# lambdaclass/mina_bridge

Measured on AMD Instinct MI355X. Metric: Mina state proofs verified/sec (batch), higher is better.
Workload: dtype u32x8-montgomery (255-bit prime fields, integer)

## Files before the change

### bindings/go/minaverify.go

```go
package minaverify

import "C"

import (
	"errors"
	"unsafe"
)

type Ctx struct{ p *C.mina_ctx }

func lastError() error { return errors.New(C.GoString(C.mina_last_error())) }

func New(device int) (*Ctx, error) {
	var p *C.mina_ctx
	if rc := C.mina_ctx_create(C.int(device), &p); rc != 0 {
		return nil, lastError()
	}
	return &Ctx{p}, nil
}

func (c *Ctx) Close() { C.mina_ctx_destroy(c.p) }

func (c *Ctx) SrsCreate(curve int, depth uint32) error {
	if rc := C.mina_srs_create(c.p, C.int(curve), C.uint32_t(depth)); rc != 0 {
// ... 18 lines not shown
	if rc := C.mina_ctx_state_dedup_stats(c.p, &a, &b, &d); rc != 0 {
		return 0, 0, 0, lastError()
	}
	return uint64(a), uint64(b), uint64(d), nil
}

func ConfigureDedupStates(otherFlags uint32) { C.mina_verify_configure(C.uint32_t(otherFlags) | C.MINA_VERIFY_DEDUP_STATES) }

func ConfigurePackOnDevice(otherFlags uint32) { C.mina_verify_configure(C.uint32_t(otherFlags) | C.MINA_VERIFY_PACK_ON_DEVICE) }

func ConfigureAccountOnDevice(otherFlags uint32) { C.mina_verify_configure(C.uint32_t(otherFlags) | C.MINA_VERIFY_ACCOUNT_ON_DEVICE) }

func ConfigureGroupedSearch(otherFlags uint32) { C.mina_verify_configure(C.uint32_t(otherFlags) | C.MINA_VERIFY_GROUPED_SEARCH) }

func (c *Ctx) SetSearchGroups(groups uint32) error {
	if rc := C.mina_ctx_set_search_groups(c.p, C.uint32_t(groups)); rc != 0 {
		return lastError()
	}
	return nil
}

func (c *Ctx) SetStreamBudget(n int) error {
	if rc := C.mina_ctx_set_stream_budget(c.p, C.int(n)); rc != 0 {
		return lastError()
	}
	return nil
}

func (c *Ctx) SearchStats() (searches, rounds, parts uint64, err error) {
	var a, b, d C.uint64_t
	if rc := C.mina_ctx_search_stats(c.p, &a, &b, &d); rc != 0 {
		return 0, 0, 0, lastError()
	}
	return uint64(a), uint64(b), uint64(d), nil
}

func (c *Ctx) StateJobEachDev(jobs *C.mina_state_jobs, dVerdicts, dFlags unsafe.Pointer) error {
	if rc := C.mina_state_job_each_dev(c.p, jobs, dVerdicts, dFlags); rc != 0 {
		return lastError()
	}
	return nil
}

func (c *Ctx) MsmSegmentsDev(curve int, nTotal, nseg int, dBegin, dEnd, dBases, dScalars, dOut unsafe.Pointer) error {
	if rc := C.mina_msm_segments_dev(c.p, C.int(curve), C.size_t(nTotal), C.size_t(nseg), dBegin, dEnd, dBases, dScalars, dOut); rc != 0 {
		return lastError()
// ... 78 lines not shown
```

### bindings/rust/src/sys.rs

```rust
#![allow(non_camel_case_types)]
use std::os::raw::{c_char, c_int, c_void};

#[repr(C)] pub struct mina_ctx { _private: [u8; 0] }

#[repr(C)]
pub struct mina_ipa_opening {
    pub k: u32,
    pub lr: *const u8,
    pub delta: *const u8,
    pub sg: *const u8,
    pub z1: *const u8,
    pub z2: *const u8,
    pub n_evalpoints: u32,
    pub evalpoints: *const u8,
    pub n_comms: u32,
    pub comms: *const u8,
    pub combined_inner_product: *const u8,
    pub polyscale: *const u8,
    pub evalscale: *const u8,
    pub sponge_state: *const u8,
    pub sponge_mode: u32,
    pub sponge_count: u32,
}

// ... 256 lines not shown
    pub fn mina_verify_account_inclusion(ctx: *mut mina_ctx, n: usize, proofs: *const *const u8, proof_lens: *const usize, pub_inputs: *const *const u8, pub_lens: *const usize, leaf_hashes: *const u8, verdicts: *mut u8) -> c_int;
    pub fn mina_consensus_project_window(p: *const mina_consensus_params, s: *const mina_consensus_state, next_global_slot: u32, out_window: *mut u32) -> c_int;
    pub fn mina_consensus_relative_min_window_density(p: *const mina_consensus_params, a: *const mina_consensus_state, b: *const mina_consensus_state, out: *mut u32) -> c_int;
    pub fn mina_consensus_is_short_range(a: *const mina_consensus_state, b: *const mina_consensus_state) -> c_int;
    pub fn mina_consensus_select_secure_chain(p: *const mina_consensus_params, tip: *const mina_consensus_state, candidate: *const mina_consensus_state, candidate_selected: *mut c_int) -> c_int;
    pub fn mina_protocol_state_pack(bytes: *const u8, len: usize, encoding: c_int, record: *mut u8, n_body_fields: *mut u32, info: *mut mina_protocol_state_info, consumed: *mut usize) -> c_int;
    pub fn mina_protocol_state_hash_batch(ctx: *mut mina_ctx, n: usize, records: *const u8, n_body_fields: *const u32, hashes_out: *mut u8, body_hashes_out: *mut u8) -> c_int;
    pub fn mina_protocol_state_dedup_dev(ctx: *mut mina_ctx, n: usize, d_records: *const c_void, d_nfields: *const c_void, d_rep: *mut c_void, d_counts: *mut c_void, fingerprint_bits: u32) -> c_int;
    pub fn mina_protocol_state_hash_batch_dedup(ctx: *mut mina_ctx, n: usize, records: *const u8, n_body_fields: *const u32, hashes_out: *mut u8, body_hashes_out: *mut u8, n_distinct: *mut usize) -> c_int;
    pub fn mina_ctx_set_state_dedup(ctx: *mut mina_ctx, on: c_int) -> c_int;
    pub fn mina_ctx_state_dedup_stats(ctx: *mut mina_ctx, states: *mut u64, distinct: *mut u64, collisions: *mut u64) -> c_int;
    pub fn mina_protocol_state_pack_dev(ctx: *mut mina_ctx, n: usize, d_blob: *const c_void, blob_len: usize, d_off: *const c_void, d_len: *const c_void, d_records: *mut c_void, d_nfields: *mut c_void, d_info: *mut c_void, d_status: *mut c_void) -> c_int;
    pub fn mina_state_frontend_dev(ctx: *mut mina_ctx, batch: usize, d_blob: *const c_void, blob_len: usize, d_begin: *const c_void, d_end: *const c_void, d_expected_hashes: *const c_void, d_ledger_hashes: *const c_void, d_and: *const c_void, d_records: *mut c_void, d_nfields: *mut c_void, d_precheck: *mut c_void, d_masks: *mut c_void) -> c_int;
    pub fn mina_protocol_state_hash_bytes(ctx: *mut mina_ctx, encoding: c_int, n: usize, states: *const *const u8, lens: *const usize, hashes_out: *mut u8) -> c_int;
    pub fn mina_state_jobs_prepare(ctx: *mut mina_ctx, log2_domain: u32, npub: u32) -> c_int;
    pub fn mina_state_job_batch_dev(ctx: *mut mina_ctx, jobs: *const mina_state_jobs, d_verdicts: *mut c_void, d_flags: *mut c_void) -> c_int;
    pub fn mina_state_job_fold_dev(ctx: *mut mina_ctx, jobs: *const mina_state_jobs, d_verdicts: *mut c_void, d_flags: *mut c_void, d_ipa_scalars: *mut c_void, d_ipa_point: *mut c_void, d_acc_scalars: *mut c_void, d_acc_point: *mut c_void) -> c_int;
    pub fn mina_state_job_batch(ctx: *mut mina_ctx, jobs: *const mina_state_jobs, verdicts: *mut u8) -> c_int;
    pub fn mina_state_job_each_dev(ctx: *mut mina_ctx, jobs: *const mina_state_jobs, d_verdicts: *mut c_void, d_flags: *mut c_void) -> c_int;
    pub fn mina_ctx_set_search_groups(ctx: *mut mina_ctx, groups: u32) -> c_int;
    pub fn mina_ctx_search_stats(ctx: *mut mina_ctx, searches: *mut u64, rounds: *mut u64, parts: *mut u64) -> c_int;
    pub fn mina_ctx_lane_streams(ctx: *mut mina_ctx, live: *mut u32, made_by_searches: *mut u64) -> c_int;
    pub fn mina_ctx_set_stream_budget(ctx: *mut mina_ctx, n: c_int) -> c_int;
    pub fn mina_challenge_to_field_dev(ctx: *mut mina_ctx, field: c_int, n: usize, d_chal128: *const c_void, d_out: *mut c_void) -> c_int;
    pub fn mina_field_sum_rows_dev(ctx: *mut mina_ctx, field: c_int, rows: usize, m: usize, d_in: *const c_void, d_out: *mut c_void) -> c_int;
    pub fn mina_msm_srs_range_dev(ctx: *mut mina_ctx, curve: c_int, first: u32, n: usize, d_scalars: *const c_void, d_out: *mut c_void) -> c_int;
    pub fn mina_msm_dev(ctx: *mut mina_ctx, curve: c_int, n: usize, d_bases: *const c_void, d_scalars: *const c_void, d_out: *mut c_void) -> c_int;
    pub fn mina_points_sum_dev(ctx: *mut mina_ctx, curve: c_int, n: usize, d_records: *const c_void, d_out: *mut c_void) -> c_int;
    pub fn mina_point_records_equal_dev(ctx: *mut mina_ctx, d_a: *const c_void, d_b: *const c_void, d_verdict: *mut c_void) -> c_int;
    pub fn mina_msm_segments_dev(ctx: *mut mina_ctx, curve: c_int, n_total: usize, nseg: usize, d_seg_begin: *const c_void, d_seg_end: *const c_void, d_bases: *const c_void, d_scalars: *const c_void, d_out: *mut c_void) -> c_int;
    pub fn mina_b_poly_fold_segments_dev(ctx: *mut mina_ctx, field: c_int, k: u32, batch: usize, nseg: usize, d_seg_begin: *const c_void, d_seg_end: *const c_void, d_chals: *const c_void, d_weights: *const c_void, d_out: *mut c_void) -> c_int;
    pub fn mina_verifier_index_install(ctx: *mut mina_ctx, index: *const mina_verifier_index) -> c_int;
    pub fn mina_verifier_index_digest(ctx: *mut mina_ctx, out32: *mut u8) -> c_int;
    pub fn mina_polish_tokens_from_json(field: c_int, json: *const c_char, len: usize, enabled_features: u32, optional_present: u32, out: *mut u8, cap: usize, out_len: *mut usize) -> c_int;
    pub fn mina_verifier_index_load_json(ctx: *mut mina_ctx, index_json: *const c_char, index_len: usize, constant_term_json: *const c_char, ct_len: usize, perm_alpha_offset: u32) -> c_int;
    pub fn mina_kimchi_to_batch(ctx: *mut mina_ctx, proofs: *const mina_kimchi_proofs, out: *mut mina_kimchi_batch_out) -> c_int;
    pub fn mina_step_index_install(ctx: *mut mina_ctx, index: *const mina_step_index) -> c_int;
    pub fn mina_step_index_load_json(ctx: *mut mina_ctx, n_indexes: usize, index_jsons: *const *const c_char, index_lens: *const usize, constant_term_json: *const c_char, ct_len: usize, enabled_features: u32, optional_present: u32) -> c_int;
    pub fn mina_pickles_public_inputs_batch(ctx: *mut mina_ctx, st: *const mina_pickles_statements, batch: usize, public_inputs_out: *mut u8, ok: *mut u8) -> c_int;
    pub fn mina_pickles_public_input(ctx: *mut mina_ctx, wrap_proof: *const u8, len: usize, encoding: c_int, app_state: *const u8, public_input_out: *mut u8, derived_out: *mut u8) -> c_int;
    pub fn mina_wrap_proof_flatten(bytes: *const u8, len: usize, encoding: c_int, out: *mut u8, cap: usize, out_len: *mut usize, consumed: *mut usize) -> c_int;
    pub fn mina_state_proof_split(bytes: *const u8, len: usize, proof_len: *mut usize, state_offsets: *mut usize, state_lens: *mut usize) -> c_int;
    pub fn mina_verify_state(proof: *const u8, proof_len: usize, pub_input: *const u8, pub_len: usize) -> bool;
    pub fn mina_verify_state_batch(n: usize, proofs: *const *const u8, proof_lens: *const usize, pub_inputs: *const *const u8, pub_lens: *const usize, verdicts_out: *mut u8) -> c_int;
    pub fn mina_verify_state_checks(proof: *const u8, proof_len: usize, pub_input: *const u8, pub_len: usize, passed_mask: *mut u32, ran_mask: *mut u32) -> c_int;
    pub fn mina_verify_state_files(proof_path: *const c_char, pub_path: *const c_char) -> bool;
// ... 30 lines not shown
```

### include/mina_verify.h

```cpp
#ifndef MINA_VERIFY_H
#define MINA_VERIFY_H

#include <stddef.h>
#include <stdint.h>

#ifdef __cplusplus
extern "C" {
#endif

#define MINA_OK 0
#define MINA_ERR_ARG (-1)
#define MINA_ERR_HIP (-2)
#define MINA_ERR_STATE (-3)
#define MINA_ERR_FORMAT (-4)

#define MINA_FIELD_FP 0
#define MINA_FIELD_FQ 1
#define MINA_CURVE_PALLAS 0
#define MINA_CURVE_VESTA 1

typedef struct mina_ctx mina_ctx;

int mina_ctx_create(int device_id, mina_ctx **out);
void mina_ctx_destroy(mina_ctx *ctx);
// ... 260 lines not shown
    const void *precheck;
    uint32_t log2_domain, npub, pub_comm_slot;
    const void *public_inputs;
    int with_ipa;
    uint32_t k, n_evalpoints, n_comms;
    const void *sponge_state , *sponge_pos , *cip , *lr , *delta ,
               *sg , *z1, *z2 , *evalpoints , *evalscale, *polyscale , *comms ;
    const void *rand_base, *sg_rand_base;
    const struct mina_kimchi_proofs *kimchi;
    int with_accumulator;
    uint32_t acc_k;
    const void *acc_prechallenges , *acc_sg , *acc_rho ;
} mina_state_jobs;
int mina_state_jobs_prepare(mina_ctx *ctx, uint32_t log2_domain, uint32_t npub);
int mina_state_job_batch_dev(mina_ctx *ctx, const mina_state_jobs *jobs, void *d_verdicts, void *d_flags);
int mina_state_job_fold_dev(mina_ctx *ctx, const mina_state_jobs *jobs, void *d_verdicts, void *d_flags, void *d_ipa_scalars, void *d_ipa_point,
                            void *d_acc_scalars, void *d_acc_point);
int mina_state_job_batch(mina_ctx *ctx, const mina_state_jobs *jobs, uint8_t *verdicts );
int mina_state_job_each_dev(mina_ctx *ctx, const mina_state_jobs *jobs, void *d_verdicts , void *d_flags );
int mina_ctx_set_search_groups(mina_ctx *ctx, uint32_t groups);
int mina_ctx_search_stats(mina_ctx *ctx, uint64_t *searches, uint64_t *rounds, uint64_t *parts);
int mina_ctx_lane_streams(mina_ctx *ctx, uint32_t *live, uint64_t *made_by_searches);
int mina_ctx_set_stream_budget(mina_ctx *ctx, int n);

int mina_challenge_to_field_dev(mina_ctx *ctx, int field, size_t n, const void *d_chal128 , void *d_out );
int mina_field_sum_rows_dev(mina_ctx *ctx, int field, size_t rows, size_t m, const void *d_in , void *d_out );
int mina_msm_srs_range_dev(mina_ctx *ctx, int curve, uint32_t first, size_t n, const void *d_scalars, void *d_out );
int mina_msm_dev(mina_ctx *ctx, int curve, size_t n, const void *d_bases , const void *d_scalars , void *d_out );
int mina_points_sum_dev(mina_ctx *ctx, int curve, size_t n, const void *d_records , void *d_out );
int mina_point_records_equal_dev(mina_ctx *ctx, const void *d_a, const void *d_b, void *d_verdict );
int mina_msm_segments_dev(mina_ctx *ctx, int curve, size_t n_total, size_t nseg, const void *d_seg_begin, const void *d_seg_end ,
                          const void *d_bases , const void *d_scalars , void *d_out );
int mina_b_poly_fold_segments_dev(mina_ctx *ctx, int field, uint32_t k, size_t batch, size_t nseg, const void *d_seg_begin,
                                  const void *d_seg_end , const void *d_chals ,
                                  const void *d_weights , void *d_out );

struct mina_pickles_statements;
#define MINA_TOK_ALPHA 0
#define MINA_TOK_BETA 1
#define MINA_TOK_GAMMA 2
#define MINA_TOK_JOINT_COMBINER 3
#define MINA_TOK_ENDO_COEFFICIENT 4
#define MINA_TOK_MDS 5
#define MINA_TOK_LITERAL 6
#define MINA_TOK_CELL 7
#define MINA_TOK_DUP 8
// ... 188 lines not shown
```

### mina_bridge_amd/csrc/api_core.hip

```cpp
#include "ctx.h"
#include "sponge.cuh"
#include "msm.cuh"

#include <sys/random.h>
#include <atomic>
#include <condition_variable>
#include <deque>
#include <mutex>

template <int F> static fe_t host_modulus() { fe_t p; for (int i = 0; i < 8; ++i) p.v[i] = modulus_limb<F>(i); return p; }
static void fe_shr1(fe_t &a) { for (int i = 0; i < 7; ++i) a.v[i] = (a.v[i] >> 1) | (a.v[i + 1] << 31); a.v[7] >>= 1; }
static fe_t fe_sub_small(const fe_t &a, uint32_t k) { fe_t r = a; uint64_t br = k; for (int i = 0; i < 8 && br; ++i) { uint64_t t = (uint64_t)r.v[i] - br; r.v[i] = (uint32_t)t; br = (t >> 32) & 1u; } return r; }
static fe_t fe_div3(const fe_t &a) { fe_t r; uint64_t rem = 0; for (int i = 7; i >= 0; --i) { uint64_t cur = (rem << 32) | a.v[i]; r.v[i] = (uint32_t)(cur / 3); rem = cur % 3; } return r; }

template <int F> static FieldK make_field_consts() {
    FieldK k;
    fe_t p = host_modulus<F>();
    fe_t a = fe_zero(); a.v[0] = 1;
    for (int i = 0; i < 512; ++i) { a = fe_add<F>(a, a); if (i == 255) k.one = a; }
    k.r2 = a;
    fe_t pm1 = fe_sub_small(p, 1);
    k.pm2 = fe_sub_small(p, 2);
    k.pm1d2 = pm1; fe_shr1(k.pm1d2);
    k.half = k.pm1d2;
// ... 65 lines not shown
    if (v->step_host && v->step_host_free && v->step_host != p->step_host) v->step_host_free(v->step_host);
    v->step_host = p->step_host; v->step_host_free = nullptr;
    v->state_salts.alias(p->state_salts); v->have_state_salts = p->have_state_salts;
}

extern "C" void mina_ctx_destroy(mina_ctx *c) {
    if (!c) return;
    (void)hipSetDevice(c->device);
    for (int i = 0; i < MB_DEV_HELPER0; ++i) if (c->lanes[i].stream) (void)hipStreamSynchronize(c->lanes[i].stream);
    for (hipStream_t s : c->fork_own) if (s) (void)hipStreamSynchronize(s);
    for (hipStream_t s : c->role) if (s) (void)hipStreamSynchronize(s);
    for (int i = 0; i < 2; ++i) { c->srs[i].table.release(); c->srs[i].table29.release(); c->srs[i].table29s.release(); c->srs[i].h.release(); c->srs[i].lagrange_table.release(); c->srs[i].lagrange_digits.release(); c->srs[i].lagrange_digits29.release(); c->pparams[i].release(); c->merkle_salts[i].release(); }
    c->state_salts.release(); c->acct_defaults.release(); c->dedup_totals.release(); c->kimchi_index.release(); c->kimchi_tokens.release(); c->kimchi_literals.release();
    c->pickles_index.release(); c->pickles_tokens.release(); c->pickles_literals.release();
    if (c->step_host && c->step_host_free) c->step_host_free(c->step_host);
    c->step_host = nullptr;
    for (int i = 0; i < MB_MAX_LANES; ++i) c->lanes[i].release_all();
    for (auto &r : c->prof.recs) { (void)hipEventDestroy(r.a); (void)hipEventDestroy(r.b); }
    for (int i = 0; i < MB_MAX_LANES; ++i) {
        Lane &L = c->lanes[i];
        if (L.aux) { (void)hipStreamSynchronize(L.aux); (void)hipStreamDestroy(L.aux); (void)hipEventDestroy(L.ev_fork); (void)hipEventDestroy(L.ev_join); }
        if (L.ev_leg) (void)hipEventDestroy(L.ev_leg);
        if (L.ev_done) (void)hipEventDestroy(L.ev_done);
        if (L.stream && i < MB_DEV_HELPER0) (void)hipStreamDestroy(L.stream);
    }
    for (hipStream_t s : c->fork_own) if (s) (void)hipStreamDestroy(s);
    for (hipStream_t s : c->role) if (s) (void)hipStreamDestroy(s);
    delete c;
}

__attribute__((constructor)) static void mb_default_hw_queues() { setenv("GPU_MAX_HW_QUEUES", "16", 0); }

extern "C" int mina_ctx_synchronize(mina_ctx *c) {
    if (!c) return fail(MINA_ERR_ARG, "null ctx");
    HIPC(hipSetDevice(c->device));
    HIPC(mb_ctx_wait_all(c));
    return MINA_OK;
}
extern "C" int mina_ctx_set_stream_budget(mina_ctx *c, int n) {
    if (!c) return fail(MINA_ERR_ARG, "null ctx");
    if (n > 31) return fail(MINA_ERR_ARG, "stream budget: at most 31 (32 hardware queues less the null stream's); <= 0 = the environment's");
    HIPC(hipSetDevice(c->device));
    HIPC(mb_ctx_wait_all(c));
    c->stream_budget = n > 0 ? n : 0;
    return MINA_OK;
}
extern "C" void *mina_ctx_stream(mina_ctx *c) { return c ? (void *)c->lanes[c->pinned >= 0 ? c->pinned : 0].stream : nullptr; }
extern "C" int mina_ctx_pin_lane(mina_ctx *c, int lane) {
    if (!c) return fail(MINA_ERR_ARG, "null ctx");
    if (lane >= c->nlanes) return fail(MINA_ERR_ARG, "lane outside the pipeline (mina_ctx_set_pipeline)");
    c->pinned = lane < 0 ? -1 : lane;
    return MINA_OK;
}

extern "C" int mina_ctx_set_pipeline(mina_ctx *c, int lanes) {
    if (!c) return fail(MINA_ERR_ARG, "null ctx");
    if (lanes < 1 || lanes > MB_PIPE_LANES) return fail(MINA_ERR_ARG, "lanes must be in 1..32");
    HIPC(hipSetDevice(c->device));
    HIPC(mb_ctx_wait_all(c));
    for (int i = 0; i < lanes; ++i)
        if (!c->lanes[i].stream) HIPC(hipStreamCreateWithFlags(&c->lanes[i].stream, hipStreamNonBlocking));
    c->nlanes = lanes; c->rr = 0; c->pinned = -1; c->use_lane0();
    return MINA_OK;
}

extern "C" int mina_to_group(mina_ctx *c, int curve, size_t n, const uint8_t *t, uint8_t *out) {
    if (!c || (n && (!t || !out))) return fail(MINA_ERR_ARG, "null argument");
// ... 180 lines not shown
```

### mina_bridge_amd/csrc/api_state.hip

```cpp
#include <chrono>
#include <optional>
#include "ctx.h"
#include "msm.cuh"
#include "sponge.cuh"
#include "lagrange.cuh"
#include "wire_state.h"
#include "state_dedup.cuh"

namespace mb {

template <int F> __device__ __forceinline__ fe_t ld_fe(const uint32_t *p) { fe_t r; for (int i = 0; i < 8; ++i) r.v[i] = p[i]; return r; }

template <int F, int LANES>
__device__ __forceinline__ void pstate_sponge(const bool live, const bool writer, const uint32_t e, const uint32_t sp, const uint32_t *__restrict__ rec, const uint32_t nf,
                                              const FieldK &fk, const PoseidonParams *__restrict__ pp, const fe_t *__restrict__ salts, uint32_t *__restrict__ out_hash,
                                              uint32_t *__restrict__ out_body) {
#if defined(__HIP_DEVICE_COMPILE__)
    if constexpr (LANES == 3) {
        const TriPos tp = tri_pos();
        const PoseidonParams29 *__restrict__ q = pparams29_of(pp);
        auto field29 = [&](const uint32_t *w, bool take) {
            fe_t v = fe_zero();
            if (take) v = ld_fe<F>(w);
            return fe29_mul_sg<F>(fe29_from_words(v), q->absorb);
// ... 186 lines not shown
static int ensure_state_salts(mina_ctx *c) {
    if (c->have_state_salts) return MINA_OK;
    if (!c->have_pparams[FIELD_FP]) return fail(MINA_ERR_STATE, "Poseidon constants not installed for Fp");
    const char *names[MB_N_PREFIX_SALTS] = {"MinaProtoStateBody", "MinaProtoState", "MinaAccount", "MinaZkappAccount", "MinaZkappUri", "MinaSideLoadedVk"};
    uint8_t pre[MB_N_PREFIX_SALTS * 32];
    for (int i = 0; i < MB_N_PREFIX_SALTS; ++i) { const mw::B32 f = mw::prefix_field(names[i]); memcpy(pre + 32 * i, f.b, 32); }
    int rc;
    if ((rc = c->state_salts.ensure(MB_N_PREFIX_SALTS * 3 * sizeof(fe_t)))) return rc;
    DevBuf tmp;
    if ((rc = tmp.ensure(sizeof pre))) return rc;
    HIPC(hipMemcpyAsync(tmp.p, pre, sizeof pre, hipMemcpyHostToDevice, c->L->stream));
    mb::prefix_salt_kernel<FIELD_FP><<<1, 64, 0, c->L->stream>>>(MB_N_PREFIX_SALTS, c->fk[FIELD_FP], c->pparams[FIELD_FP].as<PoseidonParams>(), tmp.as<uint32_t>(), c->state_salts.as<fe_t>());
    HIPC(hipGetLastError());
    HIPC(hipStreamSynchronize(c->L->stream));
    tmp.release();
    c->have_state_salts = true;
    return MINA_OK;
}

int mb_ensure_state_salts(mina_ctx *c) { return ensure_state_salts(c); }

struct UniqList { const uint32_t *m, *uniq; };
static int pstate_hash_launch(mina_ctx *c, size_t n, size_t leg, HashLaunch hl, const uint32_t *d_records, const uint32_t *d_nfields, uint32_t *d_hashes, uint32_t *d_bodies,
                              const UniqList *u) {
    const PoseidonParams *pp = c->pparams[FIELD_FP].as<PoseidonParams>();
    const fe_t *salts = c->state_salts.as<fe_t>();
    hipStream_t stream = c->L->stream;
    return with_lanes<1, 16, 8, 3>(pstate_hash_lanes(c, n, leg), [&](auto lanes) {
        constexpr int LN = decltype(lanes)::value;
        constexpr bool wide = LN == 1 || LN == 3;
        std::optional<ProfScope> ps1_;
        if (LN == 1) ps1_.emplace(c, PS_STATE_HASH1);
        const size_t per = wide && hl.piece_waves ? hash_piece_states(c, leg, hl.piece_waves) : n;
        const uint32_t lds = wide ? hl.lds_bytes : 0;
        for (size_t lo = 0; lo < n; lo += per) {
            const size_t cnt = std::min(per, n - lo);
            const uint32_t grid = cdiv(coop_threads<LN>(cnt), 256);
            if (u) {
                if constexpr (LN == 1) mb::pstate_hash1_uniq_kernel<FIELD_FP><<<grid, 256, lds, stream>>>((uint32_t)lo, (uint32_t)cnt, u->m, u->uniq, pp, salts, d_records, d_nfields, d_hashes, d_bodies);
                else mb::pstate_hash_uniq_kernel<FIELD_FP, LN><<<grid, 256, lds, stream>>>((uint32_t)lo, (uint32_t)cnt, u->m, u->uniq, c->fk[FIELD_FP], pp, salts, d_records, d_nfields, d_hashes, d_bodies);
                continue;
            }
            const uint32_t *rec = d_records + lo * MINA_PSTATE_SLOTS * 8, *nf = d_nfields + lo;
            uint32_t *hash = d_hashes + lo * 8, *body = d_bodies ? d_bodies + lo * 8 : nullptr;
            if constexpr (LN == 1) mb::pstate_hash1_kernel<FIELD_FP><<<grid, 256, lds, stream>>>((uint32_t)cnt, pp, salts, rec, nf, hash, body);
            else mb::pstate_hash_kernel<FIELD_FP, LN><<<grid, 256, lds, stream>>>((uint32_t)cnt, c->fk[FIELD_FP], pp, salts, rec, nf, hash, body);
        }
        HIPC(hipGetLastError());
        return MINA_OK;
    });
}

static int pstate_hash_dev(mina_ctx *c, size_t n, size_t leg, HashLaunch hl, const uint32_t *d_records, const uint32_t *d_nfields, uint32_t *d_hashes, uint32_t *d_bodies) {
    ProfScope ps_(c, PS_STATE_HASH);
    return pstate_hash_launch(c, n, leg, hl, d_records, d_nfields, d_hashes, d_bodies, nullptr);
}
// ... 193 lines not shown
    if (!LS || lo + cnt > ns_total) return fail(MINA_ERR_ARG, "bad early state range");
    if (!c->have_state_salts) return fail(MINA_ERR_STATE, "call mina_state_jobs_prepare first");
    if (!LS->stream) HIPC(hipStreamCreateWithFlags(&LS->stream, hipStreamNonBlocking));
    int rc;
    if ((rc = LS->st_hashes.ensure(ns_total * 32))) return rc;
    if (after) HIPC(hipStreamWaitEvent(LS->stream, after, 0));
    Lane *const L0 = c->L;
    c->L = LS;
    rc = pstate_hash_dev(c, cnt, ns_total, hash, d_records + lo * MINA_PSTATE_SLOTS * 8, d_nfields + lo, LS->st_hashes.as<uint32_t>() + lo * 8, nullptr);
    c->L = L0;
    return rc;
}


static int state_leg(mina_ctx *c, const mina_state_jobs *j, Lane &S, const StateJobPlan &plan) {
    c->L = &S;
    const size_t B = j->batch;
    int rc;
    if (j->with_states) {
        const size_t ns = B * MINA_STATES_PER_PROOF;
        if ((rc = S.st_hashes.ensure(ns * 32))) return rc;
        const size_t early = std::min(plan.hashed_early, ns);
        const uint32_t *rec = (const uint32_t *)j->state_records, *nf = (const uint32_t *)j->state_nfields;
        if (c->state_dedup && early == 0) {
            if ((rc = pstate_hash_dedup_dev(c, ns, ns, plan.hash, rec, nf, S.st_hashes.as<uint32_t>(), nullptr, true))) return rc;
        } else if (early < ns && (rc = pstate_hash_dev(c, ns - early, ns, plan.hash, rec + early * MINA_PSTATE_SLOTS * 8, nf + early, S.st_hashes.as<uint32_t>() + early * 8, nullptr))) return rc;
        mb::pstate_chain_check_kernel<<<cdiv(B, 64), 64, 0, S.stream>>>((uint32_t)B, S.st_hashes.as<uint32_t>(), (const uint32_t *)j->expected_hashes, rec, (const uint8_t *)j->precheck, S.st_ok.as<uint32_t>());
    } else {
        if (j->precheck) return fail(MINA_ERR_ARG, "precheck needs the protocol-state section");
        mb::fill_u32_kernel<<<cdiv(B, 256), 256, 0, S.stream>>>((uint32_t)B, 1u, S.st_ok.as<uint32_t>());
    }
    HIPC(hipGetLastError());
    return MINA_OK;
}

static int accumulator_leg(mina_ctx *c, const mina_state_jobs *j, Lane &A, const FoldExport *fx, StateJobCarry &v) {
    c->L = &A;
    if (!j->with_accumulator) return MINA_OK;
    const size_t B = j->batch;
    int rc;
    if ((rc = A.st_flags.ensure(16 * 4))) return rc;
    v.acc_v = A.st_flags.as<uint32_t>() + 8;
    return mb_accumulator_check_dev(c, CURVE_VESTA, j->acc_k, B, (const uint32_t *)j->acc_prechallenges, (const uint32_t *)j->acc_sg, B > 1 ? (const uint32_t *)j->acc_rho : nullptr, v.acc_v, fx);
}

static int wrap_leg(mina_ctx *c, const mina_state_jobs *j, Lane &L, const FoldExport *fx, StateJobCarry &v, hipStream_t stage2 = nullptr) {
    c->L = &L;
    const size_t B = j->batch;
// ... 140 lines not shown
    const StreamPlan sp = stream_plan(in_flight, c->stream_budget > 0 ? c->stream_budget : c->stream_budget_env);
    const uint32_t mode = c->dev_fork_made ? c->dev_fork_made : tu.dev_fork;
    c->dev_fork_made = mode;
    int prio_lo = 0, prio_hi = 0;
    auto make = [&](hipStream_t &st, bool chain, bool masked, int prio) -> int {
        if (st) return MINA_OK;
        int ncu = 0; (void)hipDeviceGetAttribute(&ncu, hipDeviceAttributeMultiprocessorCount, c->device);
        if (masked && tu.dev_chain_cus > 0 && tu.dev_chain_cus < (uint32_t)ncu && ncu <= 256) {
            uint32_t mk[8] = {0, 0, 0, 0, 0, 0, 0, 0};
            for (uint32_t b2 = 0; b2 < (uint32_t)ncu; ++b2) if ((b2 < tu.dev_chain_cus) == chain) mk[b2 >> 5] |= 1u << (b2 & 31);
            if (hipExtStreamCreateWithCUMask(&st, 8, mk) == hipSuccess) return MINA_OK;
            (void)hipGetLastError(); st = nullptr;
        }
        if (prio_lo != prio_hi && (mode & 4u)) HIPC(hipStreamCreateWithPriority(&st, hipStreamNonBlocking, prio));
        else HIPC(hipStreamCreateWithFlags(&st, hipStreamNonBlocking));
        return MINA_OK;
    };
    int rc;
    if (sp.roles) {
        if (!c->role[sp.streams - 1]) (void)hipDeviceGetStreamPriorityRange(&prio_lo, &prio_hi);
        for (int i = 0; i < sp.streams; ++i) if ((rc = make(c->role[i], true, false, (i == 0 && sp.streams > 1) ? prio_lo : prio_hi))) return rc;
        plan.role_h = c->role[0]; plan.role_w1 = c->role[sp.w1(li)]; plan.role_w2 = c->role[sp.w2(li)];
        plan.wrap = &h[0]; plan.acc = &h[1]; plan.states = &h[2];
    } else {
        hipStream_t *own = &c->fork_own[3 * li];
        if (!own[0] || !own[1] || !own[2]) {
            (void)hipDeviceGetStreamPriorityRange(&prio_lo, &prio_hi);
            if ((rc = make(own[0], true, (mode & 2u) != 0, prio_hi)) || (rc = make(own[1], true, false, (prio_lo + prio_hi) / 2)) || (rc = make(own[2], false, (mode & 2u) != 0, prio_lo))) return rc;
        }
        for (int q = 0; q < 3; ++q) h[q].stream = own[q];
        if (L0.on_roles) {
            HIPC(hipStreamWaitEvent(L0.stream, L0.ev_done, 0));
            L0.on_roles = false;
        }
        plan.wrap = &h[0]; plan.acc = tu.dev_acc_lane ? &h[2] : &h[1]; plan.states = &h[2];
        plan.acc_first = tu.dev_acc_lane == 2;
    }
    uint32_t piece = tu.dev_piece_waves;
    if (piece == 0 && in_flight >= 2 && !sp.roles) piece = (hash_one_lane(c, leg_states) ? 12288u : 6144u) / (uint32_t)in_flight;
    if (piece == 0xffffffffu) piece = 0;
    plan.hash.piece_waves = piece;
    uint32_t lds_kb = tu.dev_hash_lds_kb;
    if (lds_kb == 0 && in_flight == 1) lds_kb = 41;
    if (lds_kb == 0xffffffffu || lds_kb > 160) lds_kb = 0;
    plan.hash.lds_bytes = lds_kb * 1024u;
    return MINA_OK;
// ... 272 lines not shown
```

### mina_bridge_amd/csrc/ctx.h

```cpp
#pragma once
#include <hip/hip_runtime.h>

#include <cstdio>
#include <cstdlib>
#include <cstring>
#include <array>
#include <functional>
#include <memory>
#include <mutex>
#include <thread>
#include <algorithm>
#include <string>
#include <type_traits>
#include <utility>
#include <vector>

#include "../../include/mina_verify.h"
#include "groupmap.cuh"

using namespace mb;

struct mina_ctx;
int mb_ctx_create_view(mina_ctx *parent, mina_ctx **out);
void mb_ctx_refresh_view(mina_ctx *view, mina_ctx *parent);
// ... 50 lines not shown
    int lagrange_table_log2 = -1;
    DevBuf lagrange_digits;
    uint32_t lagrange_digits_n = 0;
    DevBuf lagrange_digits29;
};

struct MsmWorkspace {
    DevBuf scalars, points, points29 , ekey, eval, eoff, count, start, task_start, rem_pos, rem_bucket, info, sorted, partial, heavy, order, redo, ghist, stage, buckets, red_r, red_ws, red2_r, red2_w, set_total, out_words, out_xyzz, buckets29, seg_bad;
};

enum ProfStage : int { PS_DIGITS = 0, PS_SCAN, PS_SCATTER, PS_ACCUMULATE, PS_BUCKET_SUM, PS_REDUCE_A, PS_REDUCE_BC, PS_FINISH,
                       PS_BPOLY_TABLES, PS_BPOLY_FOLD, PS_BPOLY_FINISH, PS_STATE_HASH, PS_IPA_TRANSCRIPT, PS_KIMCHI, PS_PICKLES,
                       PS_STATE_HASH1 , PS_COUNT };
struct ProfState {
    int mask = 0;
    struct Rec { hipEvent_t a, b; int stage; };
    std::vector<Rec> recs; size_t used = 0;
};

struct Lane {
    hipStream_t stream = nullptr;
    hipStream_t aux = nullptr;
    hipEvent_t ev_fork = nullptr, ev_join = nullptr, ev_leg = nullptr;
    hipEvent_t ev_done = nullptr; bool on_roles = false;
    MsmWorkspace ws;
    DevBuf tmp_a, tmp_b, tmp_c, tmp_d;
    PinnedBuf host_stage;
    DevBuf bp_ltab, bp_htab, bp_partial, bp_ldig, bp_hdig, bp_colsum;
    DevBuf ipa_chals, ipa_folded, ipa_xyzz_a, ipa_xyzz_b, ipa_points, ipa_scalars, ipa_sigma, ipa_in_a, ipa_in_b, ipa_in_c, ipa_verdict, ipa_xfer, ipa_shared, ipa_shared_off, acc_rho_scaled ;
    DevBuf st_ok, st_hashes, st_pub_xyzz, st_pubcomm, st_flags, st_in, st_verdicts;
    DevBuf dd_rep, dd_uniq, dd_table, dd_counts;
    DevBuf pk_off, pk_len, pk_status, pk_info, pk_fmt;
    DevBuf ac_ws, ac_in;
    DevBuf gs_tab, gs_folded, gs_xa, gs_xb, gs_chals, gs_points, gs_bad, gs_flags;
    DevBuf kc_state, kc_pos, kc_cip, kc_pts, kc_v, kc_u, kc_comms, kc_xfer, kc_pch, pk_xe, pk_pub, pk_ok;
    void release_all() {
        MsmWorkspace &w = ws;
        DevBuf *all[] = {&w.scalars, &w.points, &w.points29, &w.ekey, &w.eval, &w.eoff, &w.count, &w.start, &w.task_start, &w.rem_pos, &w.rem_bucket, &w.info, &w.sorted, &w.partial, &w.heavy, &w.order, &w.redo, &w.ghist, &w.stage,
                         &w.buckets, &w.buckets29, &w.seg_bad, &w.red_r, &w.red_ws, &w.red2_r, &w.red2_w, &w.set_total, &w.out_words, &w.out_xyzz, &tmp_a, &tmp_b, &tmp_c, &tmp_d,
                         &bp_ltab, &bp_htab, &bp_partial, &bp_ldig, &bp_hdig, &bp_colsum, &ipa_chals, &ipa_folded, &ipa_xyzz_a, &ipa_xyzz_b, &ipa_points, &ipa_scalars,
                         &ipa_sigma, &ipa_in_a, &ipa_in_b, &ipa_in_c, &ipa_verdict, &ipa_xfer, &ipa_shared, &ipa_shared_off, &acc_rho_scaled,
                         &st_ok, &st_hashes, &st_pub_xyzz, &st_pubcomm, &st_flags, &st_in, &st_verdicts,
                         &dd_rep, &dd_uniq, &dd_table, &dd_counts, &pk_off, &pk_len, &pk_status, &pk_info, &pk_fmt, &ac_ws, &ac_in,
                         &gs_tab, &gs_folded, &gs_xa, &gs_xb, &gs_chals, &gs_points, &gs_bad, &gs_flags,
                         &kc_state, &kc_pos, &kc_cip, &kc_pts, &kc_v, &kc_u, &kc_comms, &kc_xfer, &kc_pch, &pk_xe, &pk_pub, &pk_ok};
        for (DevBuf *b : all) b->release();
// ... 39 lines not shown
    DevBuf pparams[2]; bool have_pparams[2] = {false, false};
    DevBuf merkle_salts[2]; uint32_t merkle_depth[2] = {0, 0};
    DevBuf kimchi_index, kimchi_tokens, kimchi_literals; bool have_kimchi = false; uint32_t kimchi_log2 = 0; uint8_t kimchi_digest[32] = {0};
    uint8_t kimchi_comms_host[28 * 64] = {0};
    DevBuf pickles_index, pickles_tokens, pickles_literals; bool have_pickles_dev = false, pickles_ms_valid = false;
    void *step_host = nullptr; void (*step_host_free)(void *) = nullptr;
    bool pparams_surrogate[2] = {false, false};
    bool pparams_rows1[2] = {false, false};
    DevBuf state_salts; bool have_state_salts = false;
    bool is_view = false;
    bool state_dedup = false;
    DevBuf dedup_totals; uint64_t dedup_states = 0;
    int (*state_frontend)(mina_ctx *c, size_t batch, const void *d_blob, size_t blob_len, const void *d_begin, const void *d_end, const void *d_expected_hashes,
                          const void *d_ledger_hashes, const void *d_and, void *d_records, void *d_nfields, void *d_precheck, void *d_masks) = nullptr;
    DevBuf acct_defaults; bool have_acct_defaults = false;
    int (*account_on_device)(mina_ctx *c, size_t n, const uint8_t *const *proofs, const size_t *proof_lens, const uint8_t *const *pubs, const size_t *pub_lens,
                             uint32_t *passed, uint32_t *ran, Lane *lane, std::mutex *enq_mu) = nullptr;
    uint32_t search_groups = 0; uint64_t gs_searches = 0, gs_rounds = 0, gs_parts = 0;
    uint64_t search_streams_made = 0;
    int (*state_job_each)(mina_ctx *c, const mina_state_jobs *dev_jobs, uint8_t *verdicts) = nullptr;
    uint32_t dev_fork_made = 0;
    hipStream_t fork_own[3 * MB_DEV_FORK_MAX] = {}; hipStream_t role[MB_ROLE_STREAMS] = {};
    int stream_budget = 0, stream_budget_env = -1;
    void use_lane0() { L = &lanes[0]; }
    void next_lane() { L = pinned >= 0 ? &lanes[pinned] : &lanes[rr++ % (unsigned)nlanes]; }
};

static inline hipError_t mb_ctx_wait_all(mina_ctx *c) {
    for (int i = 0; i < c->nlanes; ++i) if (c->lanes[i].stream) { hipError_t e = hipStreamSynchronize(c->lanes[i].stream); if (e != hipSuccess) return e; }
    for (hipStream_t s : c->role) if (s) { hipError_t e = hipStreamSynchronize(s); if (e != hipSuccess) return e; }
    return hipSuccess;
}

static inline int mb_ctx_state_dedup(mina_ctx *c, bool on) {
    if (on && !c->state_dedup) {
        if (mb_ctx_wait_all(c) != hipSuccess) return MINA_ERR_HIP;
        int rc = c->dedup_totals.ensure(16);
        if (rc) return rc;
        if (hipMemsetAsync(c->dedup_totals.p, 0, 16, c->lanes[0].stream) != hipSuccess || hipStreamSynchronize(c->lanes[0].stream) != hipSuccess) return MINA_ERR_HIP;
        c->dedup_states = 0;
    }
    c->state_dedup = on;
    return MINA_OK;
}

static constexpr size_t COOP8_MAX_GROUPS = 8192;
static inline bool use_coop8(const mina_ctx *c, size_t groups) {
    const mina_verify_tuning t = mb_tune();
    return groups * (size_t)((c && !t.coop8_per_call) ? c->nlanes : 1) <= (size_t)t.coop8_max;
}

static inline bool use_coop16(const mina_ctx *c, size_t proofs) {
    return proofs * (size_t)(c ? c->nlanes : 1) <= (size_t)mb_tune().coop16_max;
}

static inline bool use_coop8_transcripts(const mina_ctx *c, size_t batch, size_t per_call_limit) {
    const size_t lim = (size_t)mb_tune().transcript_coop8_max;
    const size_t in_flight = batch * (size_t)(c ? c->nlanes : 1);
    return lim ? in_flight <= lim : ((batch <= per_call_limit && in_flight <= 2048) || in_flight <= 2560);
}

static constexpr size_t HASH1_MIN_STATES = 65536;
static inline int hash_jobs_in_flight(const mina_ctx *c) { return c->pinned >= 0 ? 1 : c->nlanes; }
static inline bool hash_one_lane(const mina_ctx *c, size_t leg_states) {
    const int jobs = hash_jobs_in_flight(c);
    return c->pparams_rows1[FIELD_FP] && jobs >= 2 && leg_states * (size_t)jobs >= HASH1_MIN_STATES;
}
static inline size_t hash_piece_states(const mina_ctx *c, size_t leg_states, uint32_t piece_waves) { return (size_t)piece_waves * (hash_one_lane(c, leg_states) ? 64u : 21u); }

static inline int hash_lanes(const mina_ctx *c, size_t proofs, size_t sponges) { return use_coop16(c, proofs) ? 16 : (use_coop8(c, sponges) ? 8 : 3); }
static inline int pstate_hash_lanes(const mina_ctx *c, size_t n, size_t leg_states) {
    return hash_one_lane(c, leg_states) ? 1 : hash_lanes(c, (n + MINA_STATES_PER_PROOF - 1) / MINA_STATES_PER_PROOF, n);
}
static inline int transcript_lanes(const mina_ctx *c, size_t batch, size_t per_call_limit) {
    return use_coop16(c, batch) ? 16 : (use_coop8_transcripts(c, batch, per_call_limit) ? 8 : 3);
}
static inline int sponge_batch_lanes(size_t n) { return n <= COOP8_MAX_GROUPS ? 8 : 3; }
static inline int merkle_lanes(const mina_ctx *c, size_t paths) { return use_coop16(c, paths) ? 16 : sponge_batch_lanes(paths); }

enum : uint32_t { MB_JOB_LEGS = 1, MB_JOB_FINISH = 2, MB_JOB_ALL = 3 };
struct StateJobCarry { uint32_t *ipa_v = nullptr, *acc_v = nullptr, *kimchi_bad = nullptr; const uint32_t *stmt_ok = nullptr; };
struct HashLaunch { uint32_t piece_waves = 0, lds_bytes = 0; };
struct FoldExport { uint32_t *ipa_scalars = nullptr, *ipa_point = nullptr, *acc_scalars = nullptr, *acc_point = nullptr; };
struct StateJobPlan {
    Lane *wrap = nullptr, *acc = nullptr, *states = nullptr;
    uint32_t phase = MB_JOB_ALL; StateJobCarry *carry = nullptr;
    uint32_t *d_stmt_out = nullptr;
    size_t hashed_early = 0;
    HashLaunch hash;
    bool acc_first = false;
    hipStream_t role_h = nullptr, role_w1 = nullptr, role_w2 = nullptr;
    const FoldExport *fold_export = nullptr;
};
int mb_state_jobs_on_lane(mina_ctx *c, const mina_state_jobs *j, uint32_t *d_verdicts, uint32_t *d_flags, const StateJobPlan &plan = {});
int mb_verify_account_on(mina_ctx *c, size_t n, const uint8_t *const *proofs, const size_t *proof_lens, const uint8_t *const *pubs, const size_t *pub_lens,
                         uint32_t *passed, uint32_t *ran, Lane *lane, std::mutex *enq_mu);
int mb_state_frontend_on_lane(mina_ctx *c, size_t batch, const void *d_blob, size_t blob_len, const void *d_begin, const void *d_end, const void *d_expected_hashes,
                              const void *d_ledger_hashes, const void *d_and, void *d_records, void *d_nfields, void *d_precheck, void *d_masks);
int mb_verify_account_dev_on(mina_ctx *c, size_t n, const uint8_t *const *proofs, const size_t *proof_lens, const uint8_t *const *pubs, const size_t *pub_lens,
                             uint32_t *passed, uint32_t *ran, Lane *lane, std::mutex *enq_mu);
int mb_state_job_each_host(mina_ctx *c, const mina_state_jobs *dev_jobs, uint8_t *verdicts);
int mb_state_hashes_early(mina_ctx *c, Lane *LS, size_t ns_total, size_t lo, size_t cnt, const uint32_t *d_records, const uint32_t *d_nfields, hipEvent_t after, HashLaunch hash);

struct MbPoolJob;
std::shared_ptr<MbPoolJob> mb_pool_submit(size_t n, std::function<void(size_t)> fn);
void mb_pool_wait(const std::shared_ptr<MbPoolJob> &job);
size_t mb_pool_threads();
template <class Fn> static inline void mb_parallel_for(size_t n, Fn fn) {
    if (n < 128 || mb_pool_threads() <= 1) { for (size_t i = 0; i < n; ++i) fn(i); return; }
    mb_pool_wait(mb_pool_submit(n, std::function<void(size_t)>(fn)));
}
bool mb_secure_random(void *buf, size_t n);
// ... 79 lines not shown
```

### mina_bridge_amd/lib.py

```python
from __future__ import annotations

import ctypes
import os

import numpy as np

HERE = os.path.dirname(os.path.abspath(__file__))
LIB_PATH = os.path.join(HERE, "libminaverify.so")

FIELD_FP, FIELD_FQ = 0, 1
CURVE_PALLAS, CURVE_VESTA = 0, 1

EXPORTS = [
    "mina_ctx_create", "mina_ctx_destroy", "mina_last_error", "mina_ctx_synchronize", "mina_ctx_stream", "mina_ctx_pin_lane", "mina_ctx_set_pipeline", "mina_prof_enable", "mina_prof_read",
    "mina_dev_malloc", "mina_dev_free", "mina_dev_upload", "mina_dev_download",
    "mina_srs_create", "mina_srs_split_table", "mina_srs_load", "mina_srs_depth", "mina_srs_get_g", "mina_srs_get_h", "mina_srs_lagrange_basis", "mina_public_input_commitment", "mina_public_input_commitment_batch", "mina_combined_inner_product", "mina_srs_serialize",
    "mina_msm", "mina_msm_srs", "mina_msm_srs_range", "mina_msm_srs_multi", "mina_msm_srs_dev",
    "mina_b_poly", "mina_b_poly_coefficients", "mina_b_poly_fold", "mina_b_poly_fold_dev",
    "mina_poseidon_set_params", "mina_poseidon_params_parse", "mina_poseidon_load_params", "mina_poseidon_load_params_file", "mina_poseidon_permute", "mina_poseidon_permute_dev", "mina_poseidon_hash",
    "mina_challenge_to_field", "mina_fq_sponge_run", "mina_to_group", "mina_merkle_roots", "mina_merkle_verify_batch",
    "mina_field_mul", "mina_field_inv", "mina_field_sqrt", "mina_selftest_group_law", "mina_selftest_fe29", "mina_selftest_fe32",
    "mina_accumulator_check_batch", "mina_accumulator_check_dev", "mina_accumulator_check_multi_dev", "mina_accumulator_check_multi", "mina_ipa_batch_check",
    "mina_consensus_project_window", "mina_consensus_relative_min_window_density", "mina_consensus_is_short_range",
    "mina_protocol_state_pack", "mina_protocol_state_hash_batch", "mina_protocol_state_hash_bytes",
    "mina_protocol_state_dedup_dev", "mina_protocol_state_hash_batch_dedup", "mina_ctx_set_state_dedup", "mina_ctx_state_dedup_stats",
    "mina_protocol_state_pack_dev", "mina_state_frontend_dev", "mina_account_frontend_dev", "mina_account_job_dev",
    "mina_state_jobs_prepare", "mina_state_job_batch_dev", "mina_state_job_batch", "mina_state_job_fold_dev",
    "mina_challenge_to_field_dev", "mina_field_sum_rows_dev", "mina_msm_srs_range_dev", "mina_msm_dev", "mina_points_sum_dev", "mina_point_records_equal_dev",
    "mina_msm_segments_dev", "mina_b_poly_fold_segments_dev", "mina_state_job_each_dev", "mina_ctx_set_search_groups", "mina_ctx_search_stats", "mina_ctx_lane_streams", "mina_ctx_set_stream_budget",
    "mina_step_index_install", "mina_step_index_load_json", "mina_polish_tokens_from_json", "mina_verifier_index_load_json", "mina_pickles_public_input",
    "mina_verifier_index_install", "mina_verifier_index_digest", "mina_kimchi_to_batch", "mina_pickles_public_inputs_batch", "mina_wrap_proof_flatten", "mina_state_proof_split",
    "mina_verify_state", "mina_verify_state_batch", "mina_verify_state_checks", "mina_verify_state_files", "mina_verify_account", "mina_verify_account_batch",
    "mina_verify_account_files", "mina_verify_account_checks", "mina_verify_account_ctx", "mina_account_hash_batch", "mina_account_abi_encode", "mina_verify_configure", "mina_verify_shutdown", "mina_verify_global_ctx", "mina_poseidon_params_name",
    "mina_verify_device_count", "mina_verify_device_ctx", "mina_verify_set_network", "mina_verify_install_verifier_index", "mina_verify_install_step_index", "mina_verify_set_poseidon_params",
    "mina_poseidon_install_default_params",
    "verify_mina_state_ffi", "verify_account_inclusion_ffi", "verify_mina_state_ffi_u32", "verify_account_inclusion_ffi_u32",
    "mina_verify_tuning_default", "mina_verify_tuning_get", "mina_verify_configure_ex", "mina_verify_retired_env",
    "mina_consensus_select_secure_chain", "mina_parse_state_pub_inputs", "mina_parse_account_pub_inputs", "mina_parse_merkle_path", "mina_verify_account_inclusion",
]


class MinaError(RuntimeError):
    pass


class StatePubInputs(ctypes.Structure):
    _fields_ = [("is_state_proof_from_devnet", ctypes.c_uint8), ("bridge_tip_state_hash", ctypes.c_uint8 * 32),
                ("candidate_chain_state_hashes", (ctypes.c_uint8 * 32) * 16), ("candidate_chain_ledger_hashes", (ctypes.c_uint8 * 32) * 16)]


def combined_inner_product(field: int, evals, polyscale, evalscale, n_polys: int, n_points: int) -> np.ndarray:
    lib = load_library()
# ... 975 lines not shown
                                                 v(d_scalars or None), v(d_out)), "mina_msm_segments_dev")

    def b_poly_fold_segments_dev(self, field: int, k: int, batch: int, nseg: int, d_seg_begin: int, d_seg_end: int, d_chals: int, d_weights: int, d_out: int):
        v = ctypes.c_void_p
        self._ck(self._lib.mina_b_poly_fold_segments_dev(self._h, field, ctypes.c_uint32(k), ctypes.c_size_t(batch), ctypes.c_size_t(nseg), v(d_seg_begin), v(d_seg_end),
                                                         v(d_chals), v(d_weights or None), v(d_out)), "mina_b_poly_fold_segments_dev")

    def set_search_groups(self, groups: int):
        self._ck(self._lib.mina_ctx_set_search_groups(self._h, ctypes.c_uint32(groups)), "mina_ctx_set_search_groups")

    def search_stats(self) -> dict:
        a, b, c = ctypes.c_uint64(0), ctypes.c_uint64(0), ctypes.c_uint64(0)
        self._ck(self._lib.mina_ctx_search_stats(self._h, ctypes.byref(a), ctypes.byref(b), ctypes.byref(c)), "mina_ctx_search_stats")
        return {"searches": a.value, "rounds": b.value, "parts": c.value}

    def lane_streams(self) -> dict:
        a, b = ctypes.c_uint32(0), ctypes.c_uint64(0)
        self._ck(self._lib.mina_ctx_lane_streams(self._h, ctypes.byref(a), ctypes.byref(b)), "mina_ctx_lane_streams")
        return {"live": a.value, "made_by_searches": b.value}

    def set_stream_budget(self, n: int):
        self._ck(self._lib.mina_ctx_set_stream_budget(self._h, ctypes.c_int(n)), "mina_ctx_set_stream_budget")

    def state_job_each_dev(self, jobs, d_verdicts: int, d_flags: int = 0):
        self._ck(self._lib.mina_state_job_each_dev(self._h, ctypes.byref(jobs), ctypes.c_void_p(d_verdicts), ctypes.c_void_p(d_flags or None)), "mina_state_job_each_dev")

    def state_jobs_prepare(self, log2_domain: int, npub: int):
        self._ck(self._lib.mina_state_jobs_prepare(self._h, ctypes.c_uint32(log2_domain), ctypes.c_uint32(npub)), "mina_state_jobs_prepare")

    @staticmethod
    def make_state_jobs(batch: int, arrays: dict, **scalars):
        j = StateJobs(); keep = []
        j.batch = batch
        kimchi = scalars.pop("kimchi", None)
        if kimchi is not None:
            j.kimchi = ctypes.addressof(kimchi[0]); keep.append(kimchi)
        for name, val in scalars.items():
            setattr(j, name, val)
        for name in StateJobs.POINTER_FIELDS:
            a = arrays.get(name)
            if a is None:
                continue
            a = np.ascontiguousarray(a); keep.append(a)
            setattr(j, name, a.ctypes.data)
        return j, keep

# ... 143 lines not shown
```

Before: 286,900.

## Split state-hash leg into full-wave body and 3-lane tail on a second stream

When a state-hash leg does not divide evenly into full single-lane waves over all SIMDs, the work is split. The whole-wave body is hashed with the one-lane kernel on the main stream, and the ragged remainder is hashed with the 3-lane kernel on the w1 role stream, joined back through an event. The aim is to avoid a mostly idle tail wave. It adds a cross-stream dependency and changes how piece sizes are computed. It also adds tuning and stats entry points to the API.

After: 290,400 (median of 6 runs). 1.2% higher.

```diff
diff --git a/bindings/go/minaverify.go b/bindings/go/minaverify.go
--- a/bindings/go/minaverify.go
+++ b/bindings/go/minaverify.go
@@ -64,6 +64,13 @@
 
 func (c *Ctx) SetStreamBudget(n int) error {
 	if rc := C.mina_ctx_set_stream_budget(c.p, C.int(n)); rc != 0 {
+		return lastError()
+	}
+	return nil
+}
+
+func (c *Ctx) SetHashSplit(simds uint32) error {
+	if rc := C.mina_ctx_set_hash_split(c.p, C.uint32_t(simds)); rc != 0 {
 		return lastError()
 	}
 	return nil
diff --git a/bindings/rust/src/sys.rs b/bindings/rust/src/sys.rs
--- a/bindings/rust/src/sys.rs
+++ b/bindings/rust/src/sys.rs
@@ -302,6 +302,8 @@
     pub fn mina_ctx_search_stats(ctx: *mut mina_ctx, searches: *mut u64, rounds: *mut u64, parts: *mut u64) -> c_int;
     pub fn mina_ctx_lane_streams(ctx: *mut mina_ctx, live: *mut u32, made_by_searches: *mut u64) -> c_int;
     pub fn mina_ctx_set_stream_budget(ctx: *mut mina_ctx, n: c_int) -> c_int;
+    pub fn mina_ctx_set_hash_split(ctx: *mut mina_ctx, simds: u32) -> c_int;
+    pub fn mina_ctx_hash_split_stats(ctx: *mut mina_ctx, legs_cut: *mut u64) -> c_int;
     pub fn mina_challenge_to_field_dev(ctx: *mut mina_ctx, field: c_int, n: usize, d_chal128: *const c_void, d_out: *mut c_void) -> c_int;
     pub fn mina_field_sum_rows_dev(ctx: *mut mina_ctx, field: c_int, rows: usize, m: usize, d_in: *const c_void, d_out: *mut c_void) -> c_int;
     pub fn mina_msm_srs_range_dev(ctx: *mut mina_ctx, curve: c_int, first: u32, n: usize, d_scalars: *const c_void, d_out: *mut c_void) -> c_int;
diff --git a/include/mina_verify.h b/include/mina_verify.h
--- a/include/mina_verify.h
+++ b/include/mina_verify.h
@@ -306,6 +306,8 @@
 int mina_ctx_search_stats(mina_ctx *ctx, uint64_t *searches, uint64_t *rounds, uint64_t *parts);
 int mina_ctx_lane_streams(mina_ctx *ctx, uint32_t *live, uint64_t *made_by_searches);
 int mina_ctx_set_stream_budget(mina_ctx *ctx, int n);
+int mina_ctx_set_hash_split(mina_ctx *ctx, uint32_t simds);
+int mina_ctx_hash_split_stats(mina_ctx *ctx, uint64_t *legs_cut);
 
 int mina_challenge_to_field_dev(mina_ctx *ctx, int field, size_t n, const void *d_chal128 , void *d_out );
 int mina_field_sum_rows_dev(mina_ctx *ctx, int field, size_t rows, size_t m, const void *d_in , void *d_out );
diff --git a/mina_bridge_amd/csrc/api_core.hip b/mina_bridge_amd/csrc/api_core.hip
--- a/mina_bridge_amd/csrc/api_core.hip
+++ b/mina_bridge_amd/csrc/api_core.hip
@@ -111,6 +111,7 @@
         if (L.aux) { (void)hipStreamSynchronize(L.aux); (void)hipStreamDestroy(L.aux); (void)hipEventDestroy(L.ev_fork); (void)hipEventDestroy(L.ev_join); }
         if (L.ev_leg) (void)hipEventDestroy(L.ev_leg);
         if (L.ev_done) (void)hipEventDestroy(L.ev_done);
+        if (L.ev_split) (void)hipEventDestroy(L.ev_split);
         if (L.stream && i < MB_DEV_HELPER0) (void)hipStreamDestroy(L.stream);
     }
     for (hipStream_t s : c->fork_own) if (s) (void)hipStreamDestroy(s);
@@ -132,6 +133,17 @@
     HIPC(hipSetDevice(c->device));
     HIPC(mb_ctx_wait_all(c));
     c->stream_budget = n > 0 ? n : 0;
+    return MINA_OK;
+}
+extern "C" int mina_ctx_set_hash_split(mina_ctx *c, uint32_t simds) {
+    if (!c) return fail(MINA_ERR_ARG, "null ctx");
+    if (simds != HASH_SPLIT_OFF && simds > (1u << 20)) return fail(MINA_ERR_ARG, "hash split: a SIMD count up to 2^20, 0 = the device's, 0xffffffff = off");
+    c->hash_split = simds;
+    return MINA_OK;
+}
+extern "C" int mina_ctx_hash_split_stats(mina_ctx *c, uint64_t *legs_cut) {
+    if (!c || !legs_cut) return fail(MINA_ERR_ARG, "null argument");
+    *legs_cut = c->hash_splits;
     return MINA_OK;
 }
 extern "C" void *mina_ctx_stream(mina_ctx *c) { return c ? (void *)c->lanes[c->pinned >= 0 ? c->pinned : 0].stream : nullptr; }
diff --git a/mina_bridge_amd/csrc/api_state.hip b/mina_bridge_amd/csrc/api_state.hip
--- a/mina_bridge_amd/csrc/api_state.hip
+++ b/mina_bridge_amd/csrc/api_state.hip
@@ -232,16 +232,16 @@
 
 struct UniqList { const uint32_t *m, *uniq; };
 static int pstate_hash_launch(mina_ctx *c, size_t n, size_t leg, HashLaunch hl, const uint32_t *d_records, const uint32_t *d_nfields, uint32_t *d_hashes, uint32_t *d_bodies,
-                              const UniqList *u) {
+                              const UniqList *u, int force_lanes = 0, hipStream_t on = nullptr ) {
     const PoseidonParams *pp = c->pparams[FIELD_FP].as<PoseidonParams>();
     const fe_t *salts = c->state_salts.as<fe_t>();
-    hipStream_t stream = c->L->stream;
-    return with_lanes<1, 16, 8, 3>(pstate_hash_lanes(c, n, leg), [&](auto lanes) {
+    hipStream_t stream = on ? on : c->L->stream;
+    return with_lanes<1, 16, 8, 3>(force_lanes ? force_lanes : pstate_hash_lanes(c, n, leg), [&](auto lanes) {
         constexpr int LN = decltype(lanes)::value;
         constexpr bool wide = LN == 1 || LN == 3;
         std::optional<ProfScope> ps1_;
         if (LN == 1) ps1_.emplace(c, PS_STATE_HASH1);
-        const size_t per = wide && hl.piece_waves ? hash_piece_states(c, leg, hl.piece_waves) : n;
+        const size_t per = wide && hl.piece_waves ? (size_t)hl.piece_waves * (LN == 1 ? 64u : 21u) : n;
         const uint32_t lds = wide ? hl.lds_bytes : 0;
         for (size_t lo = 0; lo < n; lo += per) {
             const size_t cnt = std::min(per, n - lo);
@@ -481,8 +481,18 @@
         if ((rc = S.st_hashes.ensure(ns * 32))) return rc;
         const size_t early = std::min(plan.hashed_early, ns);
         const uint32_t *rec = (const uint32_t *)j->state_records, *nf = (const uint32_t *)j->state_nfields;
+        const bool split = plan.hash_body > 0 && plan.hash_body < ns && early == 0;
         if (c->state_dedup && early == 0) {
             if ((rc = pstate_hash_dedup_dev(c, ns, ns, plan.hash, rec, nf, S.st_hashes.as<uint32_t>(), nullptr, true))) return rc;
+        } else if (split) {
+            const size_t body = plan.hash_body;
+            ProfScope ps_(c, PS_STATE_HASH);
+            if ((rc = pstate_hash_launch(c, body, ns, plan.hash, rec, nf, S.st_hashes.as<uint32_t>(), nullptr, nullptr))) return rc;
+            if (!S.ev_split) HIPC(hipEventCreateWithFlags(&S.ev_split, hipEventDisableTiming));
+            if ((rc = pstate_hash_launch(c, ns - body, ns, plan.hash, rec + body * MINA_PSTATE_SLOTS * 8, nf + body, S.st_hashes.as<uint32_t>() + body * 8, nullptr, nullptr, 3, plan.role_w1))) return rc;
+            HIPC(hipEventRecord(S.ev_split, plan.role_w1));
+            HIPC(hipStreamWaitEvent(S.stream, S.ev_split, 0));
+            c->hash_splits += 1;
         } else if (early < ns && (rc = pstate_hash_dev(c, ns - early, ns, plan.hash, rec + early * MINA_PSTATE_SLOTS * 8, nf + early, S.st_hashes.as<uint32_t>() + early * 8, nullptr))) return rc;
         mb::pstate_chain_check_kernel<<<cdiv(B, 64), 64, 0, S.stream>>>((uint32_t)B, S.st_hashes.as<uint32_t>(), (const uint32_t *)j->expected_hashes, rec, (const uint8_t *)j->precheck, S.st_ok.as<uint32_t>());
     } else {
@@ -669,6 +679,11 @@
         for (int i = 0; i < sp.streams; ++i) if ((rc = make(c->role[i], true, false, (i == 0 && sp.streams > 1) ? prio_lo : prio_hi))) return rc;
         plan.role_h = c->role[0]; plan.role_w1 = c->role[sp.w1(li)]; plan.role_w2 = c->role[sp.w2(li)];
         plan.wrap = &h[0]; plan.acc = &h[1]; plan.states = &h[2];
+        if (!c->simds_dev) { int ncu = 0; (void)hipDeviceGetAttribute(&ncu, hipDeviceAttributeMultiprocessorCount, c->device); c->simds_dev = ncu > 0 ? 4u * (uint32_t)ncu : 0u; }
+        if (plan.role_h != plan.role_w1 && leg_states && !c->state_dedup && hash_one_lane(c, leg_states)) {
+            const size_t body = hash_split_body(leg_states, c->hash_split ? c->hash_split : c->simds_dev);
+            if (body < leg_states) plan.hash_body = body;
+        }
     } else {
         hipStream_t *own = &c->fork_own[3 * li];
         if (!own[0] || !own[1] || !own[2]) {
diff --git a/mina_bridge_amd/csrc/ctx.h b/mina_bridge_amd/csrc/ctx.h
--- a/mina_bridge_amd/csrc/ctx.h
+++ b/mina_bridge_amd/csrc/ctx.h
@@ -96,6 +96,7 @@
     hipStream_t stream = nullptr;
     hipStream_t aux = nullptr;
     hipEvent_t ev_fork = nullptr, ev_join = nullptr, ev_leg = nullptr;
+    hipEvent_t ev_split = nullptr;
     hipEvent_t ev_done = nullptr; bool on_roles = false;
     MsmWorkspace ws;
     DevBuf tmp_a, tmp_b, tmp_c, tmp_d;
@@ -181,6 +182,8 @@
     uint32_t dev_fork_made = 0;
     hipStream_t fork_own[3 * MB_DEV_FORK_MAX] = {}; hipStream_t role[MB_ROLE_STREAMS] = {};
     int stream_budget = 0, stream_budget_env = -1;
+    uint32_t hash_split = 0, simds_dev = 0;
+    uint64_t hash_splits = 0;
     void use_lane0() { L = &lanes[0]; }
     void next_lane() { L = pinned >= 0 ? &lanes[pinned] : &lanes[rr++ % (unsigned)nlanes]; }
 };
@@ -227,6 +230,17 @@
 }
 static inline size_t hash_piece_states(const mina_ctx *c, size_t leg_states, uint32_t piece_waves) { return (size_t)piece_waves * (hash_one_lane(c, leg_states) ? 64u : 21u); }
 
+static constexpr uint32_t HASH_SPLIT_OFF = 0xffffffffu;
+static inline size_t hash_split_body(size_t leg_states, uint32_t simds) {
+    if (simds == HASH_SPLIT_OFF || simds == 0) return leg_states;
+    const uint64_t per = 64ull * simds;
+    if (leg_states < per) return leg_states;
+    const uint64_t body = leg_states / per * per, rem = leg_states - body;
+    if (rem == 0) return leg_states;
+    if ((rem + 20) / 21 * 923ull > 2544ull * simds) return leg_states;
+    return (size_t)body;
+}
+
 static inline int hash_lanes(const mina_ctx *c, size_t proofs, size_t sponges) { return use_coop16(c, proofs) ? 16 : (use_coop8(c, sponges) ? 8 : 3); }
 static inline int pstate_hash_lanes(const mina_ctx *c, size_t n, size_t leg_states) {
     return hash_one_lane(c, leg_states) ? 1 : hash_lanes(c, (n + MINA_STATES_PER_PROOF - 1) / MINA_STATES_PER_PROOF, n);
@@ -247,6 +261,7 @@
     uint32_t *d_stmt_out = nullptr;
     size_t hashed_early = 0;
     HashLaunch hash;
+    size_t hash_body = 0;
     bool acc_first = false;
     hipStream_t role_h = nullptr, role_w1 = nullptr, role_w2 = nullptr;
     const FoldExport *fold_export = nullptr;
diff --git a/mina_bridge_amd/lib.py b/mina_bridge_amd/lib.py
--- a/mina_bridge_amd/lib.py
+++ b/mina_bridge_amd/lib.py
@@ -27,7 +27,7 @@
     "mina_protocol_state_pack_dev", "mina_state_frontend_dev", "mina_account_frontend_dev", "mina_account_job_dev",
     "mina_state_jobs_prepare", "mina_state_job_batch_dev", "mina_state_job_batch", "mina_state_job_fold_dev",
     "mina_challenge_to_field_dev", "mina_field_sum_rows_dev", "mina_msm_srs_range_dev", "mina_msm_dev", "mina_points_sum_dev", "mina_point_records_equal_dev",
-    "mina_msm_segments_dev", "mina_b_poly_fold_segments_dev", "mina_state_job_each_dev", "mina_ctx_set_search_groups", "mina_ctx_search_stats", "mina_ctx_lane_streams", "mina_ctx_set_stream_budget",
+    "mina_msm_segments_dev", "mina_b_poly_fold_segments_dev", "mina_state_job_each_dev", "mina_ctx_set_search_groups", "mina_ctx_search_stats", "mina_ctx_lane_streams", "mina_ctx_set_stream_budget", "mina_ctx_set_hash_split", "mina_ctx_hash_split_stats",
     "mina_step_index_install", "mina_step_index_load_json", "mina_polish_tokens_from_json", "mina_verifier_index_load_json", "mina_pickles_public_input",
     "mina_verifier_index_install", "mina_verifier_index_digest", "mina_kimchi_to_batch", "mina_pickles_public_inputs_batch", "mina_wrap_proof_flatten", "mina_state_proof_split",
     "mina_verify_state", "mina_verify_state_batch", "mina_verify_state_checks", "mina_verify_state_files", "mina_verify_account", "mina_verify_account_batch",
@@ -1049,6 +1049,14 @@
     def set_stream_budget(self, n: int):
         self._ck(self._lib.mina_ctx_set_stream_budget(self._h, ctypes.c_int(n)), "mina_ctx_set_stream_budget")
 
+    def set_hash_split(self, simds: int):
+        self._ck(self._lib.mina_ctx_set_hash_split(self._h, ctypes.c_uint32(simds)), "mina_ctx_set_hash_split")
+
+    def hash_split_stats(self) -> int:
+        a = ctypes.c_uint64(0)
+        self._ck(self._lib.mina_ctx_hash_split_stats(self._h, ctypes.byref(a)), "mina_ctx_hash_split_stats")
+        return int(a.value)
+
     def state_job_each_dev(self, jobs, d_verdicts: int, d_flags: int = 0):
         self._ck(self._lib.mina_state_job_each_dev(self._h, ctypes.byref(jobs), ctypes.c_void_p(d_verdicts), ctypes.c_void_p(d_flags or None)), "mina_state_job_each_dev")
 
```
